# NeurAI-Lab/biHomE

Hardware: AMD Instinct MI355X
Metric: training image-pairs/s (128x128 patch, bs=64 per GPU, full step: fwd+bwd+Adam) (higher is better)
Workload: dtype f32

## Files before the change

bihome_amd/csrc/bn.hip:

```cpp
#include "common.h"

#define BN_MAX_CHUNKS 256

struct BnGeom {
    int groups, rows, C, C4, LPR, RPP, nchunks, rows_per_chunk;
    int det;
};

static bool bn_geom(int groups, int rows, int C, BnGeom& g, int det) {
    if (C < 4 || C % 4 || groups < 1 || rows < 1) return false;
    g.groups = groups; g.rows = rows; g.C = C; g.C4 = C / 4; g.det = det;
    if (g.C4 > 256 || (256 % g.C4)) return false;
    g.LPR = g.C4; g.RPP = 256 / g.LPR;
    int n = rows / (g.RPP * 4);
    if (n < 1) n = 1;
    if (n > BN_MAX_CHUNKS) n = BN_MAX_CHUNKS;
    g.rows_per_chunk = (rows + n - 1) / n;
    g.nchunks = (rows + g.rows_per_chunk - 1) / g.rows_per_chunk;
    return true;
}

template <int NV>
__device__ __forceinline__ void reduce_rows(double (&v)[NV], int LPR, int RPP, double* sm ) {
    for (int i = 0; i < NV; ++i) sm[threadIdx.x * NV + i] = v[i];
// ... 803 lines not shown
}

__global__ void __launch_bounds__(256) bn_fwd_coeffs_kernel(const double* __restrict__ stats, const float* __restrict__ gamma,
                                                            const float* __restrict__ beta, BnGeom g, float eps, float momentum,
                                                            float* __restrict__ upd_mean, float* __restrict__ upd_var,
                                                            float2* __restrict__ table, unsigned* __restrict__ amax) {
    __shared__ float sm_amax[4];
    if (upd_mean && blockIdx.x == gridDim.x - 1) { bn_update_running(stats, g, momentum, upd_mean, upd_var); return; }
    const int i = blockIdx.x * 256 + threadIdx.x;
    float bound = 0.f;
    if (i < g.groups * g.C) {
        const int grp = i / g.C, c = i - grp * g.C;
        float mean, invstd, sc, sh;
        bn_coeffs(stats, gamma, beta, nullptr, nullptr, 0, g.groups, grp, g.C, c, eps, (double)g.rows, mean, invstd, sc, sh, g.det);
        table[i] = make_float2(sc, sh);
        bound = 2.0f * (fabsf(gamma ? gamma[c] : 1.f) * sqrtf((float)g.rows) + fabsf(beta ? beta[c] : 0.f));
    }
    if (amax) bh_amax_commit(amax, bound, blockIdx.x, sm_amax);
}

int bn_launch_stats(const float* x, int groups, int rows, int C, double* sums, hipStream_t s, int det) {
    BnGeom g;
    if (!bn_geom(groups, rows, C, g, det ? 1 : 0)) return BH_E_UNSUPPORTED;
    hipLaunchKernelGGL(bn_stats_kernel, dim3(g.nchunks, groups), dim3(256), 0, s, x, g, sums);
    BH_LAUNCH_CHECK();
    return BH_OK;
}

int bn1_fwd(const float* x, const float* gamma, const float* beta, float* running_mean, float* running_var, const float* res, float* y,
            double* stats, int groups, int rows, float eps, float momentum, int flags, int use_running, hipStream_t s);
int bn1_bwd(const float* gy, const float* y, const float* x, const float* gamma, const float* beta, const double* stats, float* gx,
            float* gres, float* ggamma, float* gbeta, double* scratch, int groups, int rows, float eps, int flags, int use_running,
            const float* running_mean, const float* running_var, hipStream_t s);

extern "C" {

int bh_bn_stats_doubles(int groups, int C) { return (int)BH_BN_SUM_DOUBLES(groups, C); }

int bh_bn_fwd(const float* x, const float* gamma, const float* beta, float* running_mean, float* running_var,
              const float* res, float* y, double* stats, int groups, int rows, int C, float eps, float momentum,
              int flags, int use_running, float* amax_y, void* stream) {
    BnGeom g;
    if (!x || !y || !stats) return BH_E_BADARG;
    if (use_running && (!running_mean || !running_var)) return BH_E_BADARG;
    if (C == 1) return amax_y ? BH_E_UNSUPPORTED : bn1_fwd(x, gamma, beta, running_mean, running_var, res, y, stats, groups, rows, eps, momentum, flags, use_running, bh_stream(stream));
    if (!bn_geom(groups, rows, C, g, (flags & BH_BN_DETERMINISTIC) ? 1 : 0)) return BH_E_UNSUPPORTED;
    hipStream_t s = bh_stream(stream);
    if (!use_running && !(flags & 8)) {
        hipLaunchKernelGGL(bn_stats_kernel, dim3(g.nchunks, groups), dim3(256), 0, s, x, g, stats);
        BH_LAUNCH_CHECK();
    }
    const bool upd = !use_running && running_mean && running_var;
    hipLaunchKernelGGL(bn_apply_kernel, dim3(apply_blocks(g), groups), dim3(256), 0, s, x, gamma, beta, running_mean,
                       running_var, res, y, stats, g, eps, flags, use_running, momentum, upd ? running_mean : nullptr,
                       upd ? running_var : nullptr, reinterpret_cast<unsigned*>(amax_y));
    BH_LAUNCH_CHECK();
    return BH_OK;
}

int bh_bn_fwd_coeffs(const double* stats, const float* gamma, const float* beta, float* running_mean, float* running_var, int groups,
                     int rows, int C, float eps, float momentum, float* table, float* amax_y, void* stream) {
    BnGeom g;
    if (!stats || !table) return BH_E_BADARG;
    if (!bn_geom(groups, rows, C, g, -1)) return BH_E_UNSUPPORTED;
    const bool upd = running_mean && running_var;
    hipLaunchKernelGGL(bn_fwd_coeffs_kernel, dim3((groups * C + 255) / 256 + (upd ? 1 : 0)), dim3(256), 0, bh_stream(stream), stats, gamma, beta, g, eps,
                       momentum, upd ? running_mean : nullptr, upd ? running_var : nullptr, reinterpret_cast<float2*>(table),
                       reinterpret_cast<unsigned*>(amax_y));
    BH_LAUNCH_CHECK();
    return BH_OK;
}

int bh_bn_bwd(const float* gy, const float* y, const float* x, const float* gamma, const float* beta, const double* stats, float* gx,
              float* gres, float* ggamma, float* gbeta, double* scratch, int groups, int rows, int C, float eps, int flags,
              int use_running, const float* running_mean, const float* running_var, float* amax_gx, void* stream) {
    BnGeom g;
    if (!gy || !x || !gx || !stats || !scratch || ((flags & 1) && !(flags & 4) && !y)) return BH_E_BADARG;
    if ((flags & 4) && (flags & 2)) return BH_E_BADARG;
    if (C == 1) return amax_gx ? BH_E_UNSUPPORTED : bn1_bwd(gy, y, x, gamma, beta, stats, gx, gres, ggamma, gbeta, scratch, groups, rows, eps, flags, use_running,
                               running_mean, running_var, bh_stream(stream));
    if (!bn_geom(groups, rows, C, g, (flags & BH_BN_DETERMINISTIC) ? 1 : 0)) return BH_E_UNSUPPORTED;
    hipStream_t s = bh_stream(stream);
    if (!use_running && rows <= BN_SMALL_ROWS) {
        hipLaunchKernelGGL(bn_bwd_small_kernel, dim3((C + 255) / 256), dim3(256), 0, s, gy, y, x, gamma, beta, stats, gx, gres, g, eps, flags,
                           ggamma, gbeta, reinterpret_cast<unsigned*>(amax_gx));
        BH_LAUNCH_CHECK();
        return BH_OK;
    }
    if (flags & 16) {
        if (use_running) return BH_E_BADARG;
        hipLaunchKernelGGL(bn_bwd_apply_kernel, dim3(apply_blocks(g), groups), dim3(256), 0, s, gy, y, x, gamma, beta,
                           (const float4*)nullptr, gx, gres, g, flags, stats, (const double*)scratch, eps, ggamma, gbeta,
                           reinterpret_cast<unsigned*>(amax_gx));
        BH_LAUNCH_CHECK();
        return BH_OK;
    }
    float4* coef = reinterpret_cast<float4*>(scratch);
    double* part = scratch + (size_t)groups * C * 2;
    const bool need_sums = !use_running || ggamma || gbeta;
    if (need_sums) {
        hipLaunchKernelGGL(bn_bwd_reduce_kernel, dim3(g.nchunks, groups), dim3(256), 0, s, gy, y, x, gamma, beta, stats,
                           running_mean, running_var, g, eps, flags, use_running, part);
        BH_LAUNCH_CHECK();
    }
    BnGeom gf = g;
    if (!need_sums) gf.nchunks = 0;
    hipLaunchKernelGGL(bn_bwd_finalize_kernel, dim3(C), dim3(64), 0, s, part, gf, stats, running_mean, running_var, eps,
                       use_running, ggamma, gbeta, coef);
    BH_LAUNCH_CHECK();
    hipLaunchKernelGGL(bn_bwd_apply_kernel, dim3(apply_blocks(g), groups), dim3(256), 0, s, gy, y, x, gamma, beta, coef,
                       gx, gres, g, flags, (const double*)nullptr, (const double*)nullptr, eps, (float*)nullptr,
                       (float*)nullptr, reinterpret_cast<unsigned*>(amax_gx));
    BH_LAUNCH_CHECK();
    return BH_OK;
}

int bh_bn_scratch_doubles(int groups, int C) { return groups * C * 2 * (1 + (BN_MAX_CHUNKS > 256 ? BN_MAX_CHUNKS : 256)); }

int bh_bn_stats(const float* x, double* stats, int groups, int rows, int C, int flags, void* stream) {
    if (!x || !stats) return BH_E_BADARG;
    return bn_launch_stats(x, groups, rows, C, stats, bh_stream(stream), (flags & BH_BN_DETERMINISTIC) ? 1 : 0);
}

int bh_bn_maxpool_fwd(const float* x, const float* gamma, const float* beta, float* running_mean, float* running_var, float* y,
                      unsigned char* idx, double* stats, int groups, int N, int Hi, int Wi, int C, float eps, float momentum, int flags,
                      int use_running, float* amax_y, void* stream) {
    BnGeom g;
    if (!x || !y || !stats || N < 1 || groups < 1 || N % groups) return BH_E_BADARG;
    if (use_running && (!running_mean || !running_var)) return BH_E_BADARG;
    const int rows = (N / groups) * Hi * Wi;
    if (!bn_geom(groups, rows, C, g, (flags & BH_BN_DETERMINISTIC) ? 1 : 0) || groups * C * 8 > 32768) return BH_E_UNSUPPORTED;
    if (rows <= BN_SMALL_ROWS) return BH_E_UNSUPPORTED;
    hipStream_t s = bh_stream(stream);
    if (!use_running && !(flags & 8)) {
        hipLaunchKernelGGL(bn_stats_kernel, dim3(g.nchunks, groups), dim3(256), 0, s, x, g, stats);
        BH_LAUNCH_CHECK();
    }
    const int Ho = (Hi - 1) / 2 + 1, Wo = (Wi - 1) / 2 + 1;
    const size_t total = (size_t)N * Ho * Wo * (C / 4);
    size_t nb = (total + 255) / 256;
    if (nb > 2048) nb = 2048;
    nb = (nb * 256 / (C / 4)) * (C / 4) / 256;
    if (nb < 1) nb = 1;
    const bool upd = !use_running && running_mean && running_var;
    hipLaunchKernelGGL(bn_maxpool_fwd_kernel, dim3((unsigned)nb), dim3(256), (size_t)groups * C * 8, s, x, gamma, beta, running_mean, running_var,
                       stats, y, idx, g, N, Hi, Wi, Ho, Wo, eps, flags & 1, use_running, momentum, upd ? running_mean : nullptr,
                       upd ? running_var : nullptr, reinterpret_cast<unsigned*>(amax_y));
    BH_LAUNCH_CHECK();
    return BH_OK;
}

struct PoolGeom { int Hi, Wi, Ho, Wo, ipg; };

struct PoolTaps {
    uchar4 w[4];
    float4 g[4];
    unsigned char t[4];
    bool ok[4];
};
__device__ __forceinline__ void pooled_taps_load(PoolTaps& q, const unsigned char* __restrict__ idx, const float* __restrict__ gy, const PoolGeom& pg,
                                                 int n, int iy, int ix, int C4, int c, bool live) {
    const int oyA = iy >> 1, oyB = (iy + 1) >> 1, oxA = ix >> 1, oxB = (ix + 1) >> 1;
    const bool vy = oyB != oyA && oyB < pg.Ho, vx = oxB != oxA && oxB < pg.Wo;
#pragma unroll
    for (int k = 0; k < 4; ++k) {
        const bool by = k >> 1, bx = k & 1;
        q.ok[k] = live && (!by || vy) && (!bx || vx);
        const int oy = (by && vy) ? oyB : oyA, ox = (bx && vx) ? oxB : oxA;
        q.t[k] = (unsigned char)((iy - (oy * 2 - 1)) * 3 + (ix - (ox * 2 - 1)));
        const size_t o = live ? (((size_t)n * pg.Ho + oy) * pg.Wo + ox) * C4 + c : 0;
        q.w[k] = *reinterpret_cast<const uchar4*>(idx + o * 4);
        q.g[k] = *reinterpret_cast<const float4*>(gy + o * 4);
    }
}
__device__ __forceinline__ float4 pooled_taps_sum(const PoolTaps& q) {
    float4 d = make_float4(0.f, 0.f, 0.f, 0.f);
#pragma unroll
    for (int k = 0; k < 4; ++k) {
        if (q.ok[k] && q.w[k].x == q.t[k]) d.x += q.g[k].x;
        if (q.ok[k] && q.w[k].y == q.t[k]) d.y += q.g[k].y;
        if (q.ok[k] && q.w[k].z == q.t[k]) d.z += q.g[k].z;
        if (q.ok[k] && q.w[k].w == q.t[k]) d.w += q.g[k].w;
    }
    return d;
}

__global__ void __launch_bounds__(256) bn_maxpool_bwd_reduce_kernel(const float* __restrict__ gy, const unsigned char* __restrict__ idx,
                                                                    const float* __restrict__ x, const float* __restrict__ gamma,
                                                                    const float* __restrict__ beta, const double* __restrict__ stats,
                                                                    const float* __restrict__ rmean, const float* __restrict__ rvar, BnGeom g,
                                                                    PoolGeom pg, float eps, int relu, int use_running, double* __restrict__ part) {
    __shared__ double sm[256 * 8];
    const int cq = threadIdx.x % g.LPR, r0 = threadIdx.x / g.LPR;
    const int grp = blockIdx.y, chunk = blockIdx.x;
    const int rbeg = chunk * g.rows_per_chunk, rend = min(g.rows, rbeg + g.rows_per_chunk);
    float mean[4], invstd[4], sc[4], sh[4];
#pragma unroll
    for (int i = 0; i < 4; ++i)
        bn_coeffs(stats, gamma, beta, rmean, rvar, use_running, g.groups, grp, g.C, cq * 4 + i, eps, (double)g.rows, mean[i], invstd[i], sc[i], sh[i], g.det);
    const size_t gbase = ((size_t)grp * g.rows) * g.C + cq * 4;
    const int hw = pg.Hi * pg.Wi;
    double v[8] = {0, 0, 0, 0, 0, 0, 0, 0};
    for (int r = rbeg + r0; r < rend; r += 4 * g.RPP) {
        float4 a[4];
        PoolTaps q[4];
#pragma unroll
        for (int u = 0; u < 4; ++u) {
            const int rr = r + u * g.RPP;
            const bool live = rr < rend;
            const int rc = live ? rr : rbeg;
            const int nl = rc / hw, p = rc - nl * hw, iy = p / pg.Wi, ix = p - iy * pg.Wi;
            a[u] = *reinterpret_cast<const float4*>(x + gbase + (size_t)rc * g.C);
            pooled_taps_load(q[u], idx, gy, pg, grp * pg.ipg + nl, iy, ix, g.C4, cq, live);
        }
#pragma unroll
        for (int u = 0; u < 4; ++u) {
            if (r + u * g.RPP >= rend) break;
            float4 d = pooled_taps_sum(q[u]);
            const float4 av = a[u];
            if (relu) {
                if (!(av.x * sc[0] + sh[0] > 0.f)) d.x = 0.f;
                if (!(av.y * sc[1] + sh[1] > 0.f)) d.y = 0.f;
                if (!(av.z * sc[2] + sh[2] > 0.f)) d.z = 0.f;
                if (!(av.w * sc[3] + sh[3] > 0.f)) d.w = 0.f;
            }
            v[0] += d.x; v[1] += d.y; v[2] += d.z; v[3] += d.w;
            v[4] += (double)(d.x * ((av.x - mean[0]) * invstd[0]));
            v[5] += (double)(d.y * ((av.y - mean[1]) * invstd[1]));
            v[6] += (double)(d.z * ((av.z - mean[2]) * invstd[2]));
            v[7] += (double)(d.w * ((av.w - mean[3]) * invstd[3]));
        }
    }
    reduce_rows<8>(v, g.LPR, g.RPP, sm);
    if ((int)threadIdx.x < g.LPR) {
        double* p = part + (((size_t)grp * g.nchunks + chunk) * g.C + cq * 4) * 2;
        for (int i = 0; i < 4; ++i) { p[i * 2] = v[i]; p[i * 2 + 1] = v[4 + i]; }
    }
}

__global__ void __launch_bounds__(256) bn_maxpool_bwd_apply_kernel(const float* __restrict__ gy, const unsigned char* __restrict__ idx,
                                                                   const float* __restrict__ x, const float* __restrict__ gamma,
                                                                   const float* __restrict__ beta, const float4* __restrict__ coef,
                                                                   float* __restrict__ gx, BnGeom g, PoolGeom pg, int relu,
                                                                   unsigned* __restrict__ amax) {
    __shared__ float sm_amax[4];
    float vmax = 0.f;
    const int cq = threadIdx.x % g.LPR, r0 = threadIdx.x / g.LPR;
    const int grp = blockIdx.y;
    float mean[4], invstd[4], sc[4], sh[4], k1[4], k2[4];
#pragma unroll
    for (int i = 0; i < 4; ++i) {
        const int c = cq * 4 + i;
        const float4 cf = coef[(size_t)grp * g.C + c];
        const float gm = gamma ? gamma[c] : 1.f, bt = beta ? beta[c] : 0.f;
        mean[i] = cf.x; invstd[i] = cf.y; k1[i] = cf.z; k2[i] = cf.w;
        sc[i] = gm * cf.y;
        sh[i] = bt - cf.x * sc[i];
    }
    const size_t gbase = ((size_t)grp * g.rows) * g.C + cq * 4;
    const int hw = pg.Hi * pg.Wi;
    const int stride = gridDim.x * g.RPP;
    for (int r = blockIdx.x * g.RPP + r0; r < g.rows; r += 4 * stride) {
        float4 a[4];
        PoolTaps q[4];
#pragma unroll
        for (int u = 0; u < 4; ++u) {
            const int rr = r + u * stride;
            const bool live = rr < g.rows;
            const int rc = live ? rr : 0;
            const int nl = rc / hw, p = rc - nl * hw, iy = p / pg.Wi, ix = p - iy * pg.Wi;
            a[u] = *reinterpret_cast<const float4*>(x + gbase + (size_t)rc * g.C);
            pooled_taps_load(q[u], idx, gy, pg, grp * pg.ipg + nl, iy, ix, g.C4, cq, live);
        }
#pragma unroll
        for (int u = 0; u < 4; ++u) {
            const int rr = r + u * stride;
            if (rr >= g.rows) break;
            float4 d = pooled_taps_sum(q[u]);
            const float4 av = a[u];
            if (relu) {
                if (!(av.x * sc[0] + sh[0] > 0.f)) d.x = 0.f;
                if (!(av.y * sc[1] + sh[1] > 0.f)) d.y = 0.f;
                if (!(av.z * sc[2] + sh[2] > 0.f)) d.z = 0.f;
                if (!(av.w * sc[3] + sh[3] > 0.f)) d.w = 0.f;
            }
            float4 o;
            o.x = sc[0] * (d.x - k1[0] - (av.x - mean[0]) * invstd[0] * k2[0]);
            o.y = sc[1] * (d.y - k1[1] - (av.y - mean[1]) * invstd[1] * k2[1]);
            o.z = sc[2] * (d.z - k1[2] - (av.z - mean[2]) * invstd[2] * k2[2]);
            o.w = sc[3] * (d.w - k1[3] - (av.w - mean[3]) * invstd[3] * k2[3]);
            *reinterpret_cast<float4*>(gx + gbase + (size_t)rr * g.C) = o;
            vmax = fmaxf(fmaxf(vmax, fmaxf(fabsf(o.x), fabsf(o.y))), fmaxf(fabsf(o.z), fabsf(o.w)));
        }
    }
    if (amax) bh_amax_commit(amax, vmax, blockIdx.x + blockIdx.y * 7u, sm_amax);
}

int bh_bn_maxpool_bwd(const float* gy, const unsigned char* idx, const float* x, const float* gamma, const float* beta, const double* stats,
                      float* gx, float* ggamma, float* gbeta, double* scratch, int groups, int N, int Hi, int Wi, int C, float eps, int flags,
                      int use_running, const float* running_mean, const float* running_var, float* amax_gx, void* stream) {
    BnGeom g;
    if (!gy || !idx || !x || !gx || !stats || !scratch || N < 1 || groups < 1 || N % groups) return BH_E_BADARG;
    if (use_running && (!running_mean || !running_var)) return BH_E_BADARG;
    const long long rows = (long long)(N / groups) * Hi * Wi;
    if (rows >= (1ll << 31) || !bn_geom(groups, (int)rows, C, g, (flags & BH_BN_DETERMINISTIC) ? 1 : 0)) return BH_E_UNSUPPORTED;
    if (rows <= BN_SMALL_ROWS) return BH_E_UNSUPPORTED;
    PoolGeom pg = {Hi, Wi, (Hi - 1) / 2 + 1, (Wi - 1) / 2 + 1, N / groups};
    hipStream_t s = bh_stream(stream);
    float4* coef = reinterpret_cast<float4*>(scratch);
    double* part = scratch + (size_t)groups * C * 2;
    const bool need_sums = !use_running || ggamma || gbeta;
    if (need_sums) {
        hipLaunchKernelGGL(bn_maxpool_bwd_reduce_kernel, dim3(g.nchunks, groups), dim3(256), 0, s, gy, idx, x, gamma, beta, stats, running_mean,
                           running_var, g, pg, eps, flags & 1, use_running, part);
        BH_LAUNCH_CHECK();
    }
    BnGeom gf = g;
    if (!need_sums) gf.nchunks = 0;
    hipLaunchKernelGGL(bn_bwd_finalize_kernel, dim3(C), dim3(64), 0, s, part, gf, stats, running_mean, running_var, eps, use_running, ggamma,
                       gbeta, coef);
    BH_LAUNCH_CHECK();
    hipLaunchKernelGGL(bn_maxpool_bwd_apply_kernel, dim3(apply_blocks(g), groups), dim3(256), 0, s, gy, idx, x, gamma, beta, coef, gx, g, pg,
                       flags & 1, reinterpret_cast<unsigned*>(amax_gx));
    BH_LAUNCH_CHECK();
    return BH_OK;
}

}

template <int KC>
__device__ __forceinline__ float4 grad_from_1x1(const float4 (&gs)[KC / 4], const float4 (&w)[KC]) {
    float4 g = make_float4(0.f, 0.f, 0.f, 0.f);
#pragma unroll
    for (int q = 0; q < KC / 4; ++q) {
        const float e[4] = {gs[q].x, gs[q].y, gs[q].z, gs[q].w};
#pragma unroll
        for (int i = 0; i < 4; ++i) {
            const float4 wk = w[q * 4 + i];
            g.x = __builtin_fmaf(e[i], wk.x, g.x); g.y = __builtin_fmaf(e[i], wk.y, g.y);
            g.z = __builtin_fmaf(e[i], wk.z, g.z); g.w = __builtin_fmaf(e[i], wk.w, g.w);
        }
    }
    return g;
}

template <int KC>
__global__ void __launch_bounds__(256) bn_bwd_1x1_reduce_kernel(const float* __restrict__ gs, const float* __restrict__ w,
                                                                const float* __restrict__ x, const float* __restrict__ gamma,
                                                                const float* __restrict__ beta, const double* __restrict__ stats, BnGeom g,
                                                                float eps, int relu, double* __restrict__ part) {
    __shared__ double sm[256 * 8];
    const int cq = threadIdx.x % g.LPR, r0 = threadIdx.x / g.LPR;
    const int grp = blockIdx.y, chunk = blockIdx.x;
    const int rbeg = chunk * g.rows_per_chunk, rend = min(g.rows, rbeg + g.rows_per_chunk);
    float4 wr[KC];
#pragma unroll
    for (int k = 0; k < KC; ++k) wr[k] = *reinterpret_cast<const float4*>(w + (size_t)k * g.C + cq * 4);
    float mean[4], invstd[4], sc[4], sh[4];
#pragma unroll
    for (int i = 0; i < 4; ++i)
        bn_coeffs(stats, gamma, beta, nullptr, nullptr, 0, g.groups, grp, g.C, cq * 4 + i, eps, (double)g.rows, mean[i], invstd[i], sc[i], sh[i], g.det);
    const size_t rbase = (size_t)grp * g.rows;
    double v[8] = {0, 0, 0, 0, 0, 0, 0, 0};
    for (int r = rbeg + r0; r < rend; r += 2 * g.RPP) {
        float4 a[2], q[2][KC / 4];
#pragma unroll
        for (int u = 0; u < 2; ++u) {
            const int rr = r + u * g.RPP;
            const size_t row = rbase + (size_t)(rr < rend ? rr : rbeg);
            a[u] = *reinterpret_cast<const float4*>(x + row * g.C + cq * 4);
#pragma unroll
            for (int j = 0; j < KC / 4; ++j) q[u][j] = *reinterpret_cast<const float4*>(gs + row * KC + j * 4);
        }
#pragma unroll
        for (int u = 0; u < 2; ++u) {
            if (r + u * g.RPP >= rend) break;
            float4 d = grad_from_1x1<KC>(q[u], wr);
            const float4 av = a[u];
            if (relu) {
                if (!(av.x * sc[0] + sh[0] > 0.f)) d.x = 0.f;
                if (!(av.y * sc[1] + sh[1] > 0.f)) d.y = 0.f;
                if (!(av.z * sc[2] + sh[2] > 0.f)) d.z = 0.f;
                if (!(av.w * sc[3] + sh[3] > 0.f)) d.w = 0.f;
            }
            v[0] += d.x; v[1] += d.y; v[2] += d.z; v[3] += d.w;
            v[4] += (double)(d.x * ((av.x - mean[0]) * invstd[0]));
            v[5] += (double)(d.y * ((av.y - mean[1]) * invstd[1]));
            v[6] += (double)(d.z * ((av.z - mean[2]) * invstd[2]));
            v[7] += (double)(d.w * ((av.w - mean[3]) * invstd[3]));
        }
    }
    reduce_rows<8>(v, g.LPR, g.RPP, sm);
    if ((int)threadIdx.x < g.LPR) {
        double* p = part + (((size_t)grp * g.nchunks + chunk) * g.C + cq * 4) * 2;
        for (int i = 0; i < 4; ++i) { p[i * 2] = v[i]; p[i * 2 + 1] = v[4 + i]; }
    }
}

template <int KC>
__global__ void __launch_bounds__(256) bn_bwd_1x1_apply_kernel(const float* __restrict__ gs, const float* __restrict__ w,
                                                               const float* __restrict__ x, const float* __restrict__ gamma,
                                                               const float* __restrict__ beta, const float4* __restrict__ coef,
                                                               float* __restrict__ gx, BnGeom g, int relu, unsigned* __restrict__ amax) {
    __shared__ float sm_amax[4];
    float vmax = 0.f;
    const int cq = threadIdx.x % g.LPR, r0 = threadIdx.x / g.LPR;
    const int grp = blockIdx.y;
    float4 wr[KC];
#pragma unroll
    for (int k = 0; k < KC; ++k) wr[k] = *reinterpret_cast<const float4*>(w + (size_t)k * g.C + cq * 4);
    float mean[4], invstd[4], sc[4], sh[4], k1[4], k2[4];
#pragma unroll
    for (int i = 0; i < 4; ++i) {
        const int c = cq * 4 + i;
        const float4 cf = coef[(size_t)grp * g.C + c];
        const float gm = gamma ? gamma[c] : 1.f, bt = beta ? beta[c] : 0.f;
        mean[i] = cf.x; invstd[i] = cf.y; k1[i] = cf.z; k2[i] = cf.w;
        sc[i] = gm * cf.y;
        sh[i] = bt - cf.x * sc[i];
    }
    const size_t rbase = (size_t)grp * g.rows;
    const int stride = gridDim.x * g.RPP;
    for (int r = blockIdx.x * g.RPP + r0; r < g.rows; r += 2 * stride) {
        float4 a[2], q[2][KC / 4];
#pragma unroll
        for (int u = 0; u < 2; ++u) {
            const int rr = r + u * stride;
            const size_t row = rbase + (size_t)(rr < g.rows ? rr : 0);
            a[u] = *reinterpret_cast<const float4*>(x + row * g.C + cq * 4);
#pragma unroll
            for (int j = 0; j < KC / 4; ++j) q[u][j] = *reinterpret_cast<const float4*>(gs + row * KC + j * 4);
        }
#pragma unroll
        for (int u = 0; u < 2; ++u) {
            const int rr = r + u * stride;
            if (rr >= g.rows) break;
            float4 d = grad_from_1x1<KC>(q[u], wr);
            const float4 av = a[u];
            if (relu) {
                if (!(av.x * sc[0] + sh[0] > 0.f)) d.x = 0.f;
                if (!(av.y * sc[1] + sh[1] > 0.f)) d.y = 0.f;
                if (!(av.z * sc[2] + sh[2] > 0.f)) d.z = 0.f;
                if (!(av.w * sc[3] + sh[3] > 0.f)) d.w = 0.f;
            }
            float4 o;
            o.x = sc[0] * (d.x - k1[0] - (av.x - mean[0]) * invstd[0] * k2[0]);
            o.y = sc[1] * (d.y - k1[1] - (av.y - mean[1]) * invstd[1] * k2[1]);
            o.z = sc[2] * (d.z - k1[2] - (av.z - mean[2]) * invstd[2] * k2[2]);
            o.w = sc[3] * (d.w - k1[3] - (av.w - mean[3]) * invstd[3] * k2[3]);
            *reinterpret_cast<float4*>(gx + (rbase + (size_t)rr) * g.C + cq * 4) = o;
            vmax = fmaxf(fmaxf(vmax, fmaxf(fabsf(o.x), fabsf(o.y))), fmaxf(fabsf(o.z), fabsf(o.w)));
        }
    }
    if (amax) bh_amax_commit(amax, vmax, blockIdx.x + blockIdx.y * 7u, sm_amax);
}

extern "C" {

// ... 95 lines not shown
```

bihome_amd/csrc/tail.hip:

```cpp
#include "common.h"

typedef float f32x2 __attribute__((ext_vector_type(2)));

#define TAIL_MAXCI 32
#define TAIL_CHUNKS 512

struct TailGeom {
    int groups, rows, hw, Ci, Cm, Co, nchunks, rows_per_chunk;
};

static bool tail_geom(int groups, int rows, int hw, int Ci, int Cm, int Co, TailGeom& g) {
    if (groups < 1 || rows < 1 || hw < 1 || Ci % 4 || Ci > TAIL_MAXCI || Ci * Ci > 256 || Cm < 64 || Cm % 64 || Cm > 256 || Co < 1 || Co > 4 ||
        rows % hw)
        return false;
    g.groups = groups; g.rows = rows; g.hw = hw; g.Ci = Ci; g.Cm = Cm; g.Co = Co;
    int n = rows / 1024;
    if (n < 1) n = 1;
    if (n > TAIL_CHUNKS) n = TAIL_CHUNKS;
    g.rows_per_chunk = (rows + n - 1) / n;
    g.nchunks = (rows + g.rows_per_chunk - 1) / g.rows_per_chunk;
    return true;
}

static inline size_t off_xmom(const TailGeom& g) { return (size_t)g.groups * g.Cm * 2; }
// ... 295 lines not shown
        for (int blk = 0; blk < NB; ++blk) {
            const float4* src = reinterpret_cast<const float4*>(w1 + (size_t)(blk * 32 + l31) * 16 + kh2 * 8);
            uint4 p0, p1, p2;
            bh_split8(src[0], src[1], p0, p1, p2);
            wpl[(blk * 3 + 0) * 64 + lane] = p0; wpl[(blk * 3 + 1) * 64 + lane] = p1; wpl[(blk * 3 + 2) * 64 + lane] = p2;
        }
    }
    __syncthreads();
    const float bo = !b2 ? 0.f : (kh2 == 0 ? b2[0] : (g.Co > 1 ? b2[1] : 0.f));
    const int nsteps = g.rows / 64, sstride = gridDim.x * 4;
    const float* xg = x + (size_t)grp * g.rows * 16 + (size_t)l31 * 16 + kh2 * 8;
    int si = blockIdx.x * 4 + wave;
    float4 xa[2], xb[2];
#pragma unroll
    for (int u = 0; u < 2; ++u) { xa[u] = make_float4(0.f, 0.f, 0.f, 0.f); xb[u] = xa[u]; }
    if (si < nsteps) {
#pragma unroll
        for (int u = 0; u < 2; ++u) {
            const float4* px = reinterpret_cast<const float4*>(xg + ((size_t)si * 64 + u * 32) * 16);
            xa[u] = px[0]; xb[u] = px[1];
        }
    }
    for (; si < nsteps; si += sstride) {
        uint4 xp[2][3];
#pragma unroll
        for (int u = 0; u < 2; ++u) bh_split8(xa[u], xb[u], xp[u][0], xp[u][1], xp[u][2]);
        const int sn = si + sstride;
        if (sn < nsteps) {
#pragma unroll
            for (int u = 0; u < 2; ++u) {
                const float4* px = reinterpret_cast<const float4*>(xg + ((size_t)sn * 64 + u * 32) * 16);
                xa[u] = px[0]; xb[u] = px[1];
            }
        }
        float o0[2] = {0.f, 0.f}, o1[2] = {0.f, 0.f};
#pragma unroll 1
        for (int blk = 0; blk < NB; ++blk) {
            const uint4 w0 = wpl[(blk * 3 + 0) * 64 + lane], wm = wpl[(blk * 3 + 1) * 64 + lane], wl = wpl[(blk * 3 + 2) * 64 + lane];
            const float4* cb = cst + blk * 32 + 4 * kh2;
            tail_f32x16 acc[2];
#pragma unroll
            for (int u = 0; u < 2; ++u) {
#pragma unroll
                for (int r = 0; r < 16; ++r) acc[u][r] = 0.f;
                acc[u] = TAIL_MFMA(wl, xp[u][0], acc[u]);
                acc[u] = TAIL_MFMA(w0, xp[u][2], acc[u]);
                acc[u] = TAIL_MFMA(wm, xp[u][1], acc[u]);
                acc[u] = TAIL_MFMA(wm, xp[u][0], acc[u]);
                acc[u] = TAIL_MFMA(w0, xp[u][1], acc[u]);
                acc[u] = TAIL_MFMA(w0, xp[u][0], acc[u]);
            }
#pragma unroll
            for (int r = 0; r < 16; ++r) {
                const float4 c = cb[(r & 3) + 8 * (r >> 2)];
#pragma unroll
                for (int u = 0; u < 2; ++u) {
                    const float t = fmaxf(fmaf(acc[u][r], c.x, c.y), 0.f);
                    o0[u] = fmaf(t, c.z, o0[u]);
                    o1[u] = fmaf(t, c.w, o1[u]);
                }
            }
        }
#pragma unroll
        for (int u = 0; u < 2; ++u) {
            const float a0 = o0[u] + __shfl_xor(o0[u], 32, 64), a1 = o1[u] + __shfl_xor(o1[u], 32, 64);
            const size_t m = (size_t)grp * g.rows + (size_t)si * 64 + u * 32 + l31;
            const size_t img = m / g.hw, p = m - img * g.hw;
            if (kh2 == 0) out[(img * g.Co) * g.hw + p] = a0 + bo;
            else if (g.Co > 1) out[(img * g.Co + 1) * g.hw + p] = a1 + bo;
        }
    }
}

template <int CI>
__global__ void __launch_bounds__(256) tail_bwd_reduce_kernel(const float* __restrict__ gout, const float* __restrict__ x,
                                                              const float* __restrict__ w1, const float* __restrict__ b1,
                                                              const float* __restrict__ gamma, const float* __restrict__ beta,
                                                              const float* __restrict__ w2, const double* __restrict__ ystats,
                                                              const float* __restrict__ rmean, const float* __restrict__ rvar,
                                                              float* __restrict__ part, TailGeom g, float eps, int use_running) {
    __shared__ __attribute__((aligned(16))) float xs[64 * CI];
    __shared__ __attribute__((aligned(16))) float gs[256 * 4];
    __shared__ int list[256];
    __shared__ int wcount[4];
    const int grp = blockIdx.y, chunk = blockIdx.x, c = threadIdx.x % g.Cm, sub = threadIdx.x / g.Cm;
    const int nsub = blockDim.x / g.Cm;
    const int rbeg = chunk * g.rows_per_chunk, rend = min(g.rows, rbeg + g.rows_per_chunk);
    const int lane = threadIdx.x & 63, wave = threadIdx.x >> 6;
    float wr[CI];
#pragma unroll
    for (int k = 0; k < CI; ++k) wr[k] = w1[c * CI + k];
    float mean, var;
    if (use_running) { mean = rmean[c]; var = rvar[c]; }
    else { mean = (float)ystats[((size_t)grp * g.Cm + c) * 2]; var = (float)ystats[((size_t)grp * g.Cm + c) * 2 + 1]; }
    const float invstd = 1.0f / sqrtf(var + eps);
    const float gm = gamma ? gamma[c] : 1.f, bt = beta ? beta[c] : 0.f, bb = b1 ? b1[c] : 0.f;
    const float scale = gm * invstd, shift = bt - mean * scale;
    float w2c[4];
    for (int o = 0; o < 4; ++o) w2c[o] = (o < g.Co) ? w2[o * g.Cm + c] : 0.f;
    float q0 = 0.f, q1 = 0.f, qz[4] = {0.f, 0.f, 0.f, 0.f}, qs[CI];
#pragma unroll
    for (int k = 0; k < CI; ++k) qs[k] = 0.f;
    const float* xbase = x + (size_t)grp * g.rows * CI;
    const int SL = blockDim.x, nwaves = (blockDim.x + 63) >> 6;
    for (int r0 = rbeg; r0 < rend; r0 += SL) {
        const int np = min(SL, rend - r0);
        __syncthreads();
        bool nzp = false;
        if ((int)threadIdx.x < np) {
            const size_t m = (size_t)grp * g.rows + r0 + threadIdx.x;
            const size_t img = m / g.hw, pp = m - img * g.hw;
            float4 gv = make_float4(0.f, 0.f, 0.f, 0.f);
            gv.x = gout[(img * g.Co) * g.hw + pp];
            if (g.Co > 1) gv.y = gout[(img * g.Co + 1) * g.hw + pp];
            if (g.Co > 2) gv.z = gout[(img * g.Co + 2) * g.hw + pp];
            if (g.Co > 3) gv.w = gout[(img * g.Co + 3) * g.hw + pp];
            reinterpret_cast<float4*>(gs)[threadIdx.x] = gv;
            nzp = gv.x != 0.f || gv.y != 0.f || gv.z != 0.f || gv.w != 0.f;
        }
        const unsigned long long bal = __ballot(nzp);
        if (lane == 0) wcount[wave] = __popcll(bal);
        __syncthreads();
        int base = 0, n = 0;
        for (int w = 0; w < nwaves; ++w) { if (w < wave) base += wcount[w]; n += wcount[w]; }
        if (n == 0) continue;
        if (nzp) list[base + __popcll(bal & ((1ull << lane) - 1ull))] = threadIdx.x;
        for (int l0 = 0; l0 < n; l0 += 64) {
            const int nn = min(64, n - l0);
            __syncthreads();
            for (int e = threadIdx.x; e < nn * (CI / 4); e += blockDim.x) {
                const int q = e / (CI / 4), f = e % (CI / 4);
                reinterpret_cast<float4*>(xs)[e] = reinterpret_cast<const float4*>(xbase + (size_t)(r0 + list[l0 + q]) * CI)[f];
            }
            __syncthreads();
            for (int q = sub; q < nn; q += nsub) {
                const float* xv = xs + q * CI;
                const float4 gq = reinterpret_cast<const float4*>(gs)[list[l0 + q]];
                float y = bb;
#pragma unroll
                for (int k = 0; k < CI; ++k) y = fmaf(wr[k], xv[k], y);
                const float yh = (y - mean) * invstd;
                const float zz = fmaf(y, scale, shift);
                const float z = fmaxf(zz, 0.f);
                const float g0 = gq.x, g1 = gq.y, g2 = gq.z, g3 = gq.w;
                float gz = g0 * w2c[0] + g1 * w2c[1] + g2 * w2c[2] + g3 * w2c[3];
                const float gbn = (zz > 0.f) ? gz : 0.f;
                q0 += gbn; q1 = fmaf(gbn, yh, q1);
                qz[0] = fmaf(g0, z, qz[0]); qz[1] = fmaf(g1, z, qz[1]); qz[2] = fmaf(g2, z, qz[2]); qz[3] = fmaf(g3, z, qz[3]);
#pragma unroll
                for (int k = 0; k < CI; ++k) qs[k] = fmaf(gbn, xv[k], qs[k]);
            }
        }
    }
    float* q = part + ((((size_t)grp * g.nchunks + chunk) * nsub + sub) * g.Cm + c) * (6 + CI);
    q[0] = q0; q[1] = q1; q[2] = qz[0]; q[3] = qz[1]; q[4] = qz[2]; q[5] = qz[3];
#pragma unroll
    for (int k = 0; k < CI; ++k) q[6 + k] = qs[k];
}

template <int CI>
__global__ void __launch_bounds__(256) tail_bwd_finalize_kernel(const float* __restrict__ part, int nsub,
                                                                const float* __restrict__ w1, const float* __restrict__ b1,
                                                                const float* __restrict__ gamma, const double* __restrict__ ws,
                                                                const float* __restrict__ rmean, const float* __restrict__ rvar,
                                                                TailGeom g, float eps, int use_running, float* __restrict__ gw1,
                                                                float* __restrict__ ggamma, float* __restrict__ gbeta,
                                                                float* __restrict__ gw2, float* __restrict__ coef) {
    __shared__ double red[4][6 + CI];
    const int c = blockIdx.x, lane = threadIdx.x & 63, wave = threadIdx.x >> 6;
    const int nm = CI + CI * CI;
    const double* ystats = ws;
    const double* xmom = ws + (size_t)g.groups * g.Cm * 2;
    const double n = (double)g.rows;
    double tgam = 0, tbet = 0, tw2[4] = {0, 0, 0, 0}, tw1 = 0;
    for (int grp = 0; grp < g.groups; ++grp) {
        double acc[6 + CI];
#pragma unroll
        for (int e = 0; e < 6 + CI; ++e) acc[e] = 0;
        for (int k = threadIdx.x; k < g.nchunks * nsub; k += 256) {
            const float* q = part + (((size_t)grp * g.nchunks * nsub + k) * g.Cm + c) * (6 + CI);
            float v[6 + CI];
#pragma unroll
            for (int e = 0; e < (6 + CI) / 2; ++e) { const float2 t = reinterpret_cast<const float2*>(q)[e]; v[2 * e] = t.x; v[2 * e + 1] = t.y; }
#pragma unroll
            for (int e = 0; e < 6 + CI; ++e) acc[e] += (double)v[e];
        }
#pragma unroll
        for (int e = 0; e < 6 + CI; ++e) acc[e] = wave_sum(acc[e]);
        __syncthreads();
        if (lane == 0) {
#pragma unroll
            for (int e = 0; e < 6 + CI; ++e) red[wave][e] = acc[e];
        }
        __syncthreads();
        if (wave == 0) {
            const double a0 = red[0][0] + red[1][0] + red[2][0] + red[3][0], a1 = red[0][1] + red[1][1] + red[2][1] + red[3][1];
            double mean, var;
            if (use_running) { mean = rmean[c]; var = rvar[c]; }
            else { mean = ystats[((size_t)grp * g.Cm + c) * 2]; var = ystats[((size_t)grp * g.Cm + c) * 2 + 1]; }
            const double invstd = 1.0 / sqrt((double)(float)var + (double)eps);
            const double gm = gamma ? (double)gamma[c] : 1.0;
            const double A = gm * invstd;
            const double kb = use_running ? 0.0 : a0 / n, kg = use_running ? 0.0 : a1 / n;
            tbet += a0; tgam += a1;
            for (int o = 0; o < 4; ++o) tw2[o] += red[0][2 + o] + red[1][2 + o] + red[2][2 + o] + red[3][2 + o];
            if (lane < CI) {
                const int k = lane;
                const double* mo = xmom + (size_t)grp * nm;
                const double sk = red[0][6 + k] + red[1][6 + k] + red[2][6 + k] + red[3][6 + k];
                if (use_running) {
                    tw1 += A * sk;
                } else {
                    double syx = ((b1 ? (double)b1[c] : 0.0) - mean) * mo[k];
                    for (int j = 0; j < CI; ++j) syx += (double)w1[c * CI + j] * mo[CI + j * CI + k];
                    syx *= invstd;
                    tw1 += A * (sk - kb * mo[k] - kg * syx);
                }
            }
            if (lane == 0) {
                float* cf = coef + ((size_t)grp * g.Cm + c) * 4;
                cf[0] = (float)A; cf[1] = (float)kb; cf[2] = (float)kg; cf[3] = 0.f;
            }
        }
    }
    if (wave == 0) {
        if (lane == 0) {
            if (ggamma) ggamma[c] += (float)tgam;
            if (gbeta) gbeta[c] += (float)tbet;
            if (gw2) for (int o = 0; o < g.Co; ++o) gw2[o * g.Cm + c] += (float)tw2[o];
        }
        if (gw1 && lane < CI) gw1[c * CI + lane] += (float)tw1;
    }
}

template <int CI>
__global__ void __launch_bounds__(256) tail_bwd_lin_kernel(const float* __restrict__ coef, const float* __restrict__ w1,
                                                           const float* __restrict__ b1, const double* __restrict__ ystats,
                                                           const float* __restrict__ rmean, const float* __restrict__ rvar, TailGeom g,
                                                           float eps, int use_running, float* __restrict__ lin) {
    constexpr int NP = 256 / CI;
    __shared__ double red[NP][CI];
    const int grp = blockIdx.y, j = blockIdx.x, k = threadIdx.x % CI, part = threadIdx.x / CI;
    const bool mat = j < CI;
    double acc = 0;
    for (int c = part; c < g.Cm; c += NP) {
        const float* cf = coef + ((size_t)grp * g.Cm + c) * 4;
        double mean, var;
        if (use_running) { mean = rmean[c]; var = rvar[c]; }
        else { mean = ystats[((size_t)grp * g.Cm + c) * 2]; var = ystats[((size_t)grp * g.Cm + c) * 2 + 1]; }
        const double invstd = 1.0 / sqrt((double)(float)var + (double)eps);
        const double A = cf[0], kb = cf[1], kg = cf[2], wk = w1[c * CI + k];
        if (mat) acc += A * kg * invstd * (double)w1[c * CI + j] * wk;
        else acc += A * (kb + kg * invstd * ((b1 ? (double)b1[c] : 0.0) - mean)) * wk;
    }
    red[part][k] = acc;
    __syncthreads();
    if (part == 0) {
        double t = 0;
        for (int q = 0; q < NP; ++q) t += red[q][k];
        lin[(size_t)grp * (CI * CI + CI) + (mat ? j * CI + k : CI * CI + k)] = (float)(-t);
    }
}

#define TAIL_SPARSE_MAX 16
template <int CI>
__global__ void __launch_bounds__(256) tail_bwd_dx_kernel(const float* __restrict__ gout, const float* __restrict__ x,
                                                          const float* __restrict__ w1, const float* __restrict__ b1,
                                                          const float* __restrict__ gamma, const float* __restrict__ beta,
                                                          const float* __restrict__ w2, const double* __restrict__ ystats,
                                                          const float* __restrict__ rmean, const float* __restrict__ rvar,
                                                          const float* __restrict__ coef, const float* __restrict__ lin,
                                                          float* __restrict__ gx, TailGeom g, float eps, int use_running) {
    extern __shared__ __attribute__((aligned(16))) float sm[];
    TailLds L;
    const int grp = blockIdx.y;
    tail_load_consts(L, sm, g, w1, b1, gamma, beta, w2, ystats, rmean, rvar, use_running, grp, eps);
    float* cf = L.mu + g.Cm;
    float* ln = cf + g.Cm * 4;
    float* w1p = ln + CI * CI + CI;
    for (int e = threadIdx.x; e < g.Cm * 4; e += 256) cf[e] = coef[(size_t)grp * g.Cm * 4 + e];
    for (int e = threadIdx.x; e < CI * CI + CI; e += 256) ln[e] = lin[(size_t)grp * (CI * CI + CI) + e];
    for (int e = threadIdx.x; e < g.Cm * CI; e += 256) w1p[(e / CI) * (CI + 1) + e % CI] = w1[e];
    __syncthreads();
    const int lane = threadIdx.x & 63;
    for (int rb = blockIdx.x * 256 + (threadIdx.x & ~63); rb < g.rows; rb += gridDim.x * 256) {
        const int r = rb + lane;
        const bool valid = r < g.rows;
        const size_t m = (size_t)grp * g.rows + (valid ? r : rb);
        float xv[CI], gxv[CI];
        load_x<CI>(x + m * CI, xv);
        const size_t img = m / g.hw, p = m - img * g.hw;
        const float* gp = gout + img * g.Co * g.hw + p;
        const float g0 = gp[0], g1 = g.Co > 1 ? gp[(size_t)g.hw] : 0.f, g2 = g.Co > 2 ? gp[2 * (size_t)g.hw] : 0.f,
                    g3 = g.Co > 3 ? gp[3 * (size_t)g.hw] : 0.f;
        int zo = 0;
        asm volatile("" : "+v"(zo));
        const float* lz = ln + zo;
#pragma unroll
        for (int k = 0; k < CI; ++k) gxv[k] = lz[CI * CI + k];
#pragma unroll
        for (int j = 0; j < CI; ++j)
#pragma unroll
            for (int k = 0; k < CI; ++k) gxv[k] = fmaf(lz[j * CI + k], xv[j], gxv[k]);
        const bool nzl = valid && (g0 != 0.f || g1 != 0.f || g2 != 0.f || g3 != 0.f);
        unsigned long long mask = __ballot(nzl);
        if (mask) {
            if (__popcll(mask) > TAIL_SPARSE_MAX) {
                for (int c = 0; c < g.Cm; ++c) {
                    const float* wr = L.w1 + c * CI;
                    const float* cs = L.cst + c * 8;
                    float y = cs[0];
#pragma unroll
                    for (int k = 0; k < CI; ++k) y = fmaf(wr[k], xv[k], y);
                    const float zz = fmaf(y, cs[1], cs[2]);
                    const float gz = g0 * cs[3] + g1 * cs[4] + g2 * cs[5] + g3 * cs[6];
                    const float gy = (zz > 0.f) ? cf[c * 4] * gz : 0.f;
#pragma unroll
                    for (int k = 0; k < CI; ++k) gxv[k] = fmaf(gy, wr[k], gxv[k]);
                }
            } else {
                while (mask) {
                    const int src = __ffsll((long long)mask) - 1;
                    mask &= mask - 1;
                    float xs_[CI];
#pragma unroll
                    for (int k = 0; k < CI; ++k) xs_[k] = __shfl(xv[k], src, 64);
                    const float s0 = __shfl(g0, src, 64), s1 = __shfl(g1, src, 64), s2 = __shfl(g2, src, 64), s3 = __shfl(g3, src, 64);
                    float acc[CI];
#pragma unroll
                    for (int k = 0; k < CI; ++k) acc[k] = 0.f;
                    for (int c = lane; c < g.Cm; c += 64) {
                        const float* wr = w1p + c * (CI + 1);
                        const float* cs = L.cst + c * 8;
// ... 288 lines not shown
```

Baseline: 5325.

## Streamline BN-maxpool backward indexing and pipeline loads; transpose tail partial layout

The BN+maxpool backward kernels swap per-row integer divisions for an incrementally stepped (n,y,x) position. Tap offsets are now computed from one base plus conditional deltas, and the tap sum uses selects instead of branches. The reduce kernel drops its 4-way unroll for 2-row double-buffered software pipelining, prefetching the next pair while the current one is summed. Separately, the tail backward partials are transposed so each channel's chunk partials are contiguous, with float2 stores, giving the finalize kernel coalesced reads. These aim to cut ALU and index overhead and improve memory access, at the cost of more register pressure and extra overflow guards.

```diff
diff --git a/bihome_amd/csrc/bn.hip b/bihome_amd/csrc/bn.hip
--- a/bihome_amd/csrc/bn.hip
+++ b/bihome_amd/csrc/bn.hip
@@ -979,23 +979,20 @@
 
 struct PoolGeom { int Hi, Wi, Ho, Wo, ipg; };
 
-struct PoolTaps {
-    uchar4 w[4];
-    float4 g[4];
-    unsigned char t[4];
-    bool ok[4];
-};
+struct PoolTaps { uchar4 w[4]; float4 g[4]; unsigned char t[4]; bool ok[4]; };
 __device__ __forceinline__ void pooled_taps_load(PoolTaps& q, const unsigned char* __restrict__ idx, const float* __restrict__ gy, const PoolGeom& pg,
                                                  int n, int iy, int ix, int C4, int c, bool live) {
-    const int oyA = iy >> 1, oyB = (iy + 1) >> 1, oxA = ix >> 1, oxB = (ix + 1) >> 1;
-    const bool vy = oyB != oyA && oyB < pg.Ho, vx = oxB != oxA && oxB < pg.Wo;
+    const int oy = iy >> 1, ox = ix >> 1, py = iy & 1, px = ix & 1;
+    const bool vy = live && py && oy + 1 < pg.Ho, vx = live && px && ox + 1 < pg.Wo;
+    const unsigned rowC4 = (unsigned)pg.Wo * (unsigned)C4, dx = vx ? (unsigned)C4 : 0u, dy = vy ? rowC4 : 0u;
+    const size_t o0 = live ? (size_t)(unsigned)(n * pg.Ho + oy) * rowC4 + (unsigned)(ox * C4 + c) : 0;
+    const int ty = (py + 1) * 3, tx = px + 1;
+    q.t[0] = (unsigned char)(ty + tx); q.t[1] = (unsigned char)ty; q.t[2] = (unsigned char)tx; q.t[3] = 0;
 #pragma unroll
     for (int k = 0; k < 4; ++k) {
         const bool by = k >> 1, bx = k & 1;
         q.ok[k] = live && (!by || vy) && (!bx || vx);
-        const int oy = (by && vy) ? oyB : oyA, ox = (bx && vx) ? oxB : oxA;
-        q.t[k] = (unsigned char)((iy - (oy * 2 - 1)) * 3 + (ix - (ox * 2 - 1)));
-        const size_t o = live ? (((size_t)n * pg.Ho + oy) * pg.Wo + ox) * C4 + c : 0;
+        const size_t o = o0 + (bx ? dx : 0u) + (by ? dy : 0u);
         q.w[k] = *reinterpret_cast<const uchar4*>(idx + o * 4);
         q.g[k] = *reinterpret_cast<const float4*>(gy + o * 4);
     }
@@ -1004,59 +1001,69 @@
     float4 d = make_float4(0.f, 0.f, 0.f, 0.f);
 #pragma unroll
     for (int k = 0; k < 4; ++k) {
-        if (q.ok[k] && q.w[k].x == q.t[k]) d.x += q.g[k].x;
-        if (q.ok[k] && q.w[k].y == q.t[k]) d.y += q.g[k].y;
-        if (q.ok[k] && q.w[k].z == q.t[k]) d.z += q.g[k].z;
-        if (q.ok[k] && q.w[k].w == q.t[k]) d.w += q.g[k].w;
+        d.x += (q.ok[k] && q.w[k].x == q.t[k]) ? q.g[k].x : -0.0f;
+        d.y += (q.ok[k] && q.w[k].y == q.t[k]) ? q.g[k].y : -0.0f;
+        d.z += (q.ok[k] && q.w[k].z == q.t[k]) ? q.g[k].z : -0.0f;
+        d.w += (q.ok[k] && q.w[k].w == q.t[k]) ? q.g[k].w : -0.0f;
     }
     return d;
 }
-
+struct PoolPos { int n, y, x; };
+__device__ __forceinline__ PoolPos pool_pos(int r, const PoolGeom& pg) {
+    PoolPos p; p.n = r / (pg.Hi * pg.Wi); const int q = r - p.n * (pg.Hi * pg.Wi); p.y = q / pg.Wi; p.x = q - p.y * pg.Wi;
+    return p;
+}
+__device__ __forceinline__ void pool_pos_add(PoolPos& p, const PoolPos& s, const PoolGeom& pg) {
+    p.x += s.x; const int cx = p.x >= pg.Wi ? 1 : 0; p.x -= cx ? pg.Wi : 0;
+    p.y += s.y + cx; const int cy = p.y >= pg.Hi ? 1 : 0; p.y -= cy ? pg.Hi : 0; p.n += s.n + cy;
+}
 __global__ void __launch_bounds__(256) bn_maxpool_bwd_reduce_kernel(const float* __restrict__ gy, const unsigned char* __restrict__ idx,
-                                                                    const float* __restrict__ x, const float* __restrict__ gamma,
-                                                                    const float* __restrict__ beta, const double* __restrict__ stats,
-                                                                    const float* __restrict__ rmean, const float* __restrict__ rvar, BnGeom g,
-                                                                    PoolGeom pg, float eps, int relu, int use_running, double* __restrict__ part) {
+                                                                    const float* __restrict__ x, const float* __restrict__ gamma, const float* __restrict__ beta,
+                                                                    const double* __restrict__ stats, const float* __restrict__ rmean, const float* __restrict__ rvar,
+                                                                    BnGeom g, PoolGeom pg, float eps, int relu, int use_running, double* __restrict__ part) {
     __shared__ double sm[256 * 8];
-    const int cq = threadIdx.x % g.LPR, r0 = threadIdx.x / g.LPR;
-    const int grp = blockIdx.y, chunk = blockIdx.x;
+    const int cq = threadIdx.x % g.LPR, r0 = threadIdx.x / g.LPR, grp = blockIdx.y, chunk = blockIdx.x;
     const int rbeg = chunk * g.rows_per_chunk, rend = min(g.rows, rbeg + g.rows_per_chunk);
     float mean[4], invstd[4], sc[4], sh[4];
 #pragma unroll
     for (int i = 0; i < 4; ++i)
         bn_coeffs(stats, gamma, beta, rmean, rvar, use_running, g.groups, grp, g.C, cq * 4 + i, eps, (double)g.rows, mean[i], invstd[i], sc[i], sh[i], g.det);
-    const size_t gbase = ((size_t)grp * g.rows) * g.C + cq * 4;
-    const int hw = pg.Hi * pg.Wi;
+    const float* const xg = x + ((size_t)grp * g.rows) * g.C + cq * 4;
+    PoolPos pos = pool_pos(rbeg + r0, pg), step = pool_pos(g.RPP, pg);
+    size_t xo = (size_t)(rbeg + r0) * g.C;
     double v[8] = {0, 0, 0, 0, 0, 0, 0, 0};
-    for (int r = rbeg + r0; r < rend; r += 4 * g.RPP) {
-        float4 a[4];
-        PoolTaps q[4];
-#pragma unroll
-        for (int u = 0; u < 4; ++u) {
-            const int rr = r + u * g.RPP;
-            const bool live = rr < rend;
-            const int rc = live ? rr : rbeg;
-            const int nl = rc / hw, p = rc - nl * hw, iy = p / pg.Wi, ix = p - iy * pg.Wi;
-            a[u] = *reinterpret_cast<const float4*>(x + gbase + (size_t)rc * g.C);
-            pooled_taps_load(q[u], idx, gy, pg, grp * pg.ipg + nl, iy, ix, g.C4, cq, live);
-        }
-#pragma unroll
-        for (int u = 0; u < 4; ++u) {
+    auto load2 = [&](int r, float4 (&a)[2], PoolTaps (&q)[2]) {
+#pragma unroll
+        for (int u = 0; u < 2; ++u, xo += (size_t)g.RPP * g.C) {
+            const bool live = r + u * g.RPP < rend;
+            a[u] = *reinterpret_cast<const float4*>(xg + (live ? xo : (size_t)rbeg * g.C));
+            pooled_taps_load(q[u], idx, gy, pg, grp * pg.ipg + pos.n, pos.y, pos.x, g.C4, cq, live);
+            pool_pos_add(pos, step, pg);
+        }
+    };
+    auto sum2 = [&](int r, const float4 (&a)[2], const PoolTaps (&q)[2]) {
+#pragma unroll
+        for (int u = 0; u < 2; ++u) {
             if (r + u * g.RPP >= rend) break;
-            float4 d = pooled_taps_sum(q[u]);
-            const float4 av = a[u];
-            if (relu) {
-                if (!(av.x * sc[0] + sh[0] > 0.f)) d.x = 0.f;
-                if (!(av.y * sc[1] + sh[1] > 0.f)) d.y = 0.f;
-                if (!(av.z * sc[2] + sh[2] > 0.f)) d.z = 0.f;
-                if (!(av.w * sc[3] + sh[3] > 0.f)) d.w = 0.f;
+            const float4 d4 = pooled_taps_sum(q[u]);
+            const float dv[4] = {d4.x, d4.y, d4.z, d4.w}, av[4] = {a[u].x, a[u].y, a[u].z, a[u].w};
+#pragma unroll
+            for (int i = 0; i < 4; ++i) {
+                const float d = (relu && !(av[i] * sc[i] + sh[i] > 0.f)) ? 0.f : dv[i];
+                v[i] += d;
+                v[4 + i] += (double)(d * ((av[i] - mean[i]) * invstd[i]));
             }
-            v[0] += d.x; v[1] += d.y; v[2] += d.z; v[3] += d.w;
-            v[4] += (double)(d.x * ((av.x - mean[0]) * invstd[0]));
-            v[5] += (double)(d.y * ((av.y - mean[1]) * invstd[1]));
-            v[6] += (double)(d.z * ((av.z - mean[2]) * invstd[2]));
-            v[7] += (double)(d.w * ((av.w - mean[3]) * invstd[3]));
-        }
+        }
+    };
+    float4 aA[2], aB[2];
+    PoolTaps qA[2], qB[2];
+    int r = rbeg + r0, pair = 2 * g.RPP;
+    load2(r, aA, qA);
+    for (; r < rend; r += 2 * pair) {
+        load2(r + pair, aB, qB);
+        sum2(r, aA, qA);
+        load2(r + 2 * pair, aA, qA);
+        sum2(r + pair, aB, qB);
     }
     reduce_rows<8>(v, g.LPR, g.RPP, sm);
     if ((int)threadIdx.x < g.LPR) {
@@ -1066,56 +1073,47 @@
 }
 
 __global__ void __launch_bounds__(256) bn_maxpool_bwd_apply_kernel(const float* __restrict__ gy, const unsigned char* __restrict__ idx,
-                                                                   const float* __restrict__ x, const float* __restrict__ gamma,
-                                                                   const float* __restrict__ beta, const float4* __restrict__ coef,
-                                                                   float* __restrict__ gx, BnGeom g, PoolGeom pg, int relu,
+                                                                   const float* __restrict__ x, const float* __restrict__ gamma, const float* __restrict__ beta,
+                                                                   const float4* __restrict__ coef, float* __restrict__ gx, BnGeom g, PoolGeom pg, int relu,
                                                                    unsigned* __restrict__ amax) {
     __shared__ float sm_amax[4];
     float vmax = 0.f;
-    const int cq = threadIdx.x % g.LPR, r0 = threadIdx.x / g.LPR;
-    const int grp = blockIdx.y;
+    const int cq = threadIdx.x % g.LPR, r0 = threadIdx.x / g.LPR, grp = blockIdx.y;
     float mean[4], invstd[4], sc[4], sh[4], k1[4], k2[4];
 #pragma unroll
     for (int i = 0; i < 4; ++i) {
-        const int c = cq * 4 + i;
-        const float4 cf = coef[(size_t)grp * g.C + c];
+        const int c = cq * 4 + i; const float4 cf = coef[(size_t)grp * g.C + c];
         const float gm = gamma ? gamma[c] : 1.f, bt = beta ? beta[c] : 0.f;
         mean[i] = cf.x; invstd[i] = cf.y; k1[i] = cf.z; k2[i] = cf.w;
-        sc[i] = gm * cf.y;
-        sh[i] = bt - cf.x * sc[i];
+        sc[i] = gm * cf.y; sh[i] = bt - cf.x * sc[i];
     }
     const size_t gbase = ((size_t)grp * g.rows) * g.C + cq * 4;
-    const int hw = pg.Hi * pg.Wi;
     const int stride = gridDim.x * g.RPP;
+    PoolPos pos = pool_pos(blockIdx.x * g.RPP + r0, pg);
+    const PoolPos step = pool_pos(stride, pg);
     for (int r = blockIdx.x * g.RPP + r0; r < g.rows; r += 4 * stride) {
         float4 a[4];
         PoolTaps q[4];
 #pragma unroll
         for (int u = 0; u < 4; ++u) {
-            const int rr = r + u * stride;
-            const bool live = rr < g.rows;
-            const int rc = live ? rr : 0;
-            const int nl = rc / hw, p = rc - nl * hw, iy = p / pg.Wi, ix = p - iy * pg.Wi;
-            a[u] = *reinterpret_cast<const float4*>(x + gbase + (size_t)rc * g.C);
-            pooled_taps_load(q[u], idx, gy, pg, grp * pg.ipg + nl, iy, ix, g.C4, cq, live);
+            const int rr = r + u * stride; const bool live = rr < g.rows;
+            a[u] = *reinterpret_cast<const float4*>(x + gbase + (size_t)(live ? rr : 0) * g.C);
+            pooled_taps_load(q[u], idx, gy, pg, grp * pg.ipg + pos.n, pos.y, pos.x, g.C4, cq, live);
+            pool_pos_add(pos, step, pg);
         }
 #pragma unroll
         for (int u = 0; u < 4; ++u) {
             const int rr = r + u * stride;
             if (rr >= g.rows) break;
-            float4 d = pooled_taps_sum(q[u]);
-            const float4 av = a[u];
-            if (relu) {
-                if (!(av.x * sc[0] + sh[0] > 0.f)) d.x = 0.f;
-                if (!(av.y * sc[1] + sh[1] > 0.f)) d.y = 0.f;
-                if (!(av.z * sc[2] + sh[2] > 0.f)) d.z = 0.f;
-                if (!(av.w * sc[3] + sh[3] > 0.f)) d.w = 0.f;
+            const float4 d4 = pooled_taps_sum(q[u]);
+            const float dv[4] = {d4.x, d4.y, d4.z, d4.w}, av[4] = {a[u].x, a[u].y, a[u].z, a[u].w};
+            float ov[4];
+#pragma unroll
+            for (int i = 0; i < 4; ++i) {
+                const float d = (relu && !(av[i] * sc[i] + sh[i] > 0.f)) ? 0.f : dv[i];
+                ov[i] = sc[i] * (d - k1[i] - (av[i] - mean[i]) * invstd[i] * k2[i]);
             }
-            float4 o;
-            o.x = sc[0] * (d.x - k1[0] - (av.x - mean[0]) * invstd[0] * k2[0]);
-            o.y = sc[1] * (d.y - k1[1] - (av.y - mean[1]) * invstd[1] * k2[1]);
-            o.z = sc[2] * (d.z - k1[2] - (av.z - mean[2]) * invstd[2] * k2[2]);
-            o.w = sc[3] * (d.w - k1[3] - (av.w - mean[3]) * invstd[3] * k2[3]);
+            const float4 o = make_float4(ov[0], ov[1], ov[2], ov[3]);
             *reinterpret_cast<float4*>(gx + gbase + (size_t)rr * g.C) = o;
             vmax = fmaxf(fmaxf(vmax, fmaxf(fabsf(o.x), fabsf(o.y))), fmaxf(fabsf(o.z), fabsf(o.w)));
         }
@@ -1130,7 +1128,7 @@
     if (!gy || !idx || !x || !gx || !stats || !scratch || N < 1 || groups < 1 || N % groups) return BH_E_BADARG;
     if (use_running && (!running_mean || !running_var)) return BH_E_BADARG;
     const long long rows = (long long)(N / groups) * Hi * Wi;
-    if (rows >= (1ll << 31) || !bn_geom(groups, (int)rows, C, g, (flags & BH_BN_DETERMINISTIC) ? 1 : 0)) return BH_E_UNSUPPORTED;
+    if (rows >= (1ll << 31) || (long long)N * Hi >= (1ll << 31) || (long long)Wi * C >= (1ll << 31) || !bn_geom(groups, (int)rows, C, g, (flags & BH_BN_DETERMINISTIC) ? 1 : 0)) return BH_E_UNSUPPORTED;
     if (rows <= BN_SMALL_ROWS) return BH_E_UNSUPPORTED;
     PoolGeom pg = {Hi, Wi, (Hi - 1) / 2 + 1, (Wi - 1) / 2 + 1, N / groups};
     hipStream_t s = bh_stream(stream);
diff --git a/bihome_amd/csrc/tail.hip b/bihome_amd/csrc/tail.hip
--- a/bihome_amd/csrc/tail.hip
+++ b/bihome_amd/csrc/tail.hip
@@ -471,10 +471,10 @@
             }
         }
     }
-    float* q = part + ((((size_t)grp * g.nchunks + chunk) * nsub + sub) * g.Cm + c) * (6 + CI);
-    q[0] = q0; q[1] = q1; q[2] = qz[0]; q[3] = qz[1]; q[4] = qz[2]; q[5] = qz[3];
-#pragma unroll
-    for (int k = 0; k < CI; ++k) q[6 + k] = qs[k];
+    float2* q = reinterpret_cast<float2*>(part + ((((size_t)grp * g.Cm + c) * g.nchunks + chunk) * nsub + sub) * (6 + CI));
+    q[0] = make_float2(q0, q1); q[1] = make_float2(qz[0], qz[1]); q[2] = make_float2(qz[2], qz[3]);
+#pragma unroll
+    for (int k = 0; k < CI; k += 2) q[3 + k / 2] = make_float2(qs[k], qs[k + 1]);
 }
 
 template <int CI>
@@ -497,7 +497,7 @@
 #pragma unroll
         for (int e = 0; e < 6 + CI; ++e) acc[e] = 0;
         for (int k = threadIdx.x; k < g.nchunks * nsub; k += 256) {
-            const float* q = part + (((size_t)grp * g.nchunks * nsub + k) * g.Cm + c) * (6 + CI);
+            const float* q = part + (((size_t)grp * g.Cm + c) * g.nchunks * nsub + k) * (6 + CI);
             float v[6 + CI];
 #pragma unroll
             for (int e = 0; e < (6 + CI) / 2; ++e) { const float2 t = reinterpret_cast<const float2*>(q)[e]; v[2 * e] = t.x; v[2 * e + 1] = t.y; }
```

New measurement: 5337 (median of 6 runs). Within noise of the previous version (+0.2%).
